# bistromath/gr-ais

Hardware: AMD Instinct MI355X
Metric: complex MS/s through corr_est->msk_timing chain; corr_est %HBM roofline (higher is better)
Workload: dtype f32

## Files before the change

### gr-ais_amd/ais_amd/_lib.py

```python
import ctypes as C
import os

_PKG = os.path.dirname(os.path.abspath(__file__))
LIB_VARIANT = os.environ.get("AISX_LIB_VARIANT", "")
LIB_PATH = os.path.join(os.path.dirname(_PKG), "lib", "libaisx_exp.so" if LIB_VARIANT == "exp" else "libaisx.so")

AISX_OK = 0
AISX_ERR_INVALID = -1
AISX_ERR_OUT_OF_RANGE = -2
AISX_ERR_HIP = -3
AISX_ERR_NO_DEVICE = -4
AISX_ERR_OVERFLOW = -5
AISX_ERR_RUNTIME = -6

AISX_FMT_CF32, AISX_FMT_CS16, AISX_FMT_CS8, AISX_FMT_CU8 = 0, 1, 2, 3
AISX_RX_ST_HDLC_OVERFLOW, AISX_RX_ST_NMEA_OVERFLOW, AISX_RX_ST_BAD_COUNT = 0x100, 0x200, 0x400
AISX_MSG_NA, AISX_MSG_STR = -(1 << 31), 48
AISX_HDLC_MAX_RULES = 16
AISX_HDLC_EV_SINGLE, AISX_HDLC_EV_PAIR, AISX_HDLC_EV_SKIP = 1, 2, 4
AISX_MLSE_ST_BAD_COUNT = 1
MLSE_BLOCK, MLSE_OVERLAP = 64, 16
AISX_MSG_FL_COMPLETE, AISX_MSG_FL_NO_LAYOUT, AISX_MSG_FL_BAD_RECORD = 1, 2, 4
AISX_NMEA_PARSE_REF_TAIL = 1
AISX_NMEAP_NAMES = ("FOUND", "KEPT", "BAD_INPUT", "LINES", "SENTENCES", "REJ_FORMAT", "REJ_CHECKSUM", "REJ_CHANNEL",
# ... 73 lines not shown
    sig("aisx_corr_set_lds_claim", i32, [vp, i32])
    sig("aisx_corr_get_lds_claim", i32, [vp, pi32, pi32])
    sig("aisx_corr_set_profiling", i32, [vp, i32])
    sig("aisx_corr_last_kernel_ms", i32, [vp, C.POINTER(C.c_float)])
    sig("aisx_corr_kernel_ms_history", i32, [vp, C.POINTER(C.c_float), i32, pi32])
    sig("aisx_corr_tags_device", i32, [vp, pvp, pvp, pi32])
    sig("aisx_corr_read_tags", i32, [vp, vp, i32, pi32, vp])
    sig("aisx_corr_read_tags_back", i32, [vp, i32, vp, i32, pi32, vp])
    sig("aisx_corr_work_host", i32, [vp, vp, vp, vp, i32, u64, vp, i32, pi32])
    sig("aisx_msk_create", i32, [pvp, f32, f32, f32, i32, i32, i32])
    sig("aisx_msk_destroy", i32, [vp])
    sig("aisx_msk_set_gain", i32, [vp, f32])
    sig("aisx_msk_get_gain", f32, [vp])
    sig("aisx_msk_set_limit", i32, [vp, f32])
    sig("aisx_msk_get_limit", f32, [vp])
    sig("aisx_msk_set_sps", i32, [vp, f32])
    sig("aisx_msk_get_sps", f32, [vp])
    sig("aisx_msk_forecast", i32, [vp, i32])
    sig("aisx_msk_out_capacity", i32, [vp])
    sig("aisx_msk_reset", i32, [vp])
    sig("aisx_msk_process_stream", i32, [vp, vp, lng, i32, vp, vp, i32, vp, vp, vp, vp, lng, vp, vp])
    sig("aisx_msk_process_stream_after", i32, [vp, vp, lng, i32, vp, vp, i32, vp, vp, vp, vp, lng, vp, vp, vp])
    sig("aisx_msk_last_status", i32, [vp, pi32, vp])
    sig("aisx_msk_restart_stats", i32, [vp, vp, vp])
    sig("aisx_msk_set_profiling", i32, [vp, i32])
    sig("aisx_msk_kernel_ms_history", i32, [vp, C.POINTER(C.c_float), i32, pi32])
    sig("aisx_msk_set_max_noutput_items", i32, [vp, i32])
    sig("aisx_msk_set_time_parallel", i32, [vp, i32, i32, i32])
    sig("aisx_msk_get_max_noutput_items", i32, [vp])
    sig("aisx_msk_set_tail_stream", i32, [vp, vp, i32])
    sig("aisx_msk_wait_tail", i32, [vp, vp])
    sig("aisx_msk_set_fused_tail", i32, [vp, i32])
    sig("aisx_msk_get_fused_tail", i32, [vp])
    sig("aisx_msk_last_tail_fused", i32, [vp])
    sig("aisx_msk_wait_prepass", i32, [vp, vp])
    sig("aisx_msk_set_head_start", i32, [vp, i32])
    sig("aisx_msk_geometry", i32, [vp, pi32, pi32])
    sig("aisx_msk_general_work_host", i32, [vp, i32, i32, vp, vp, vp, vp, vp, vp, i32, u64, i32, pi32, pi32])
    sig("aisx_freqsync_create", i32, [pvp, f64, f64, i32, i32, i32])
    sig("aisx_freqest_create", i32, [pvp, f32, i32, i32, i32])
    sig("aisx_freqest_create_n", i32, [pvp, f32, i32, i32, i32, i32])
    sig("aisx_freqsync_is_estimator_only", i32, [vp])
    sig("aisx_freqsync_geometry", i32, [vp, pi32, pi32, pi32])
    sig("aisx_freqsync_drop_ahead", i32, [vp, vp])
    sig("aisx_freqsync_destroy", i32, [vp])
    sig("aisx_freqsync_reset", i32, [vp])
    sig("aisx_freqsync_process", i32, [vp, vp, lng, i32, vp, lng, vp, lng, pi32, vp])
    sig("aisx_freqest_work", i32, [vp, vp, lng, vp, lng, i32, vp])
    sig("aisx_freqest_work_host", i32, [vp, i32, vp, vp])
    sig("aisx_freqsync_work_host", i32, [vp, vp, i32, vp, i32, vp, i32])
    sig("aisx_agc_work_host", i32, [vp, i32, vp, vp])
    sig("aisx_freqsync_agc_process", i32, [vp, vp, vp, lng, i32, vp, lng, vp, lng, pi32, vp])
    sig("aisx_freqsync_estimate_ahead", i32, [vp, vp, lng, i32, vp, vp])
    sig("aisx_agc_create", i32, [pvp, i32, f32, i32, i32])
    sig("aisx_agc_destroy", i32, [vp])
    sig("aisx_agc_geometry", i32, [vp, pi32, pi32, pi32, pi32])
    sig("aisx_agc_reset", i32, [vp])
    sig("aisx_agc_set_floor", i32, [vp, f32])
    sig("aisx_agc_set_streaming", i32, [vp, i32])
    sig("aisx_agc_set_lds_claim", i32, [vp, i32])
    sig("aisx_agc_get_lds_claim", i32, [vp, pi32, pi32])
    sig("aisx_freqsync_set_walk_lds_claim", i32, [vp, i32])
    sig("aisx_freqsync_get_walk_lds_claim", i32, [vp, pi32, pi32])
    sig("aisx_msk_placement", i32, [vp, pi32, pi32])
    sig("aisx_agc_process", i32, [vp, vp, lng, vp, lng, i32, vp])
    sig("aisx_chain_create", i32, [pvp, vp, vp, vp, vp, i32, i32, i32])
# ... 138 lines not shown
```

### gr-ais_amd/ais_amd/blocks.py

```python
import ctypes as C
import math

import numpy as np
import torch

from . import _lib
from ._lib import check

TAG_DTYPE = np.dtype([("offset", "<u8"), ("value", "<f8"), ("key", "<i4"), ("chan", "<i4")])


def _stream_ptr(stream=None):
    s = stream if stream is not None else torch.cuda.current_stream()
    return C.c_void_p(s.cuda_stream)


def _dev_c64(x, nchan):
    if not isinstance(x, torch.Tensor):
        x = torch.as_tensor(np.ascontiguousarray(x, dtype=np.complex64))
    if x.dtype != torch.complex64:
        raise TypeError("expected complex64 (gr_complex) items, got %s" % x.dtype)
    if not x.is_cuda:
        x = x.cuda()
    x = x.reshape(nchan, -1)
# ... 190 lines not shown
            else:
                width = min(width, t.shape[1])
        if prod.dim() != 1 or prod.shape[0] < self.nchan or prod.dtype != torch.int32 or not prod.is_cuda:
            raise ValueError("msk_timing_recovery_cc.work: outs['produced'] must be an int32 device tensor of nchan items")
        if stride is None:
            stride = width = cap
        if width < stride:
            raise ValueError("msk_timing_recovery_cc.work: output rows must be as wide as their stride")
        if tags_ptrs is not None:
            tptr, cptr, tcap = tags_ptrs
        elif tags_from is not None:
            tptr, cptr, tcap = tags_from.tags_device()
        else:
            tptr, cptr, tcap = None, None, 0
        check(_lib.lib().aisx_msk_process_stream(
            self._h, x.data_ptr(), x.stride(0), n, tptr, cptr, tcap,
            syms.data_ptr() if syms is not None else None, err.data_ptr() if err is not None else None,
            mu.data_ptr() if mu is not None else None, bits.data_ptr() if bits is not None else None, stride,
            prod.data_ptr(), _stream_ptr(stream)), "msk_timing_recovery_cc.work")
        return dict(syms=syms, err=err, mu=mu, bits=bits, produced=prod)

    def set_tail_stream(self, stream):
        check(_lib.lib().aisx_msk_set_tail_stream(self._h, _stream_ptr(stream) if stream is not None else None,
                                                  1 if stream is not None else 0), "set_tail_stream")

    def wait_tail(self, stream=None):
        check(_lib.lib().aisx_msk_wait_tail(self._h, _stream_ptr(stream)), "wait_tail")

    def set_fused_tail(self, on):
        check(_lib.lib().aisx_msk_set_fused_tail(self._h, 1 if on else 0), "set_fused_tail")

    def get_fused_tail(self):
        return bool(_lib.lib().aisx_msk_get_fused_tail(self._h))

    def last_tail_fused(self):
        return _lib.lib().aisx_msk_last_tail_fused(self._h) == 1

    def wait_prepass(self, stream=None):
        check(_lib.lib().aisx_msk_wait_prepass(self._h, _stream_ptr(stream)), "wait_prepass")

    def last_status(self, stream=None):
        st = C.c_int(0)
        check(_lib.lib().aisx_msk_last_status(self._h, C.byref(st), _stream_ptr(stream)), "last_status")
        return st.value

    def set_time_parallel(self, restart_points=64, join_kernel=-1, max_unit_items=0):
        check(_lib.lib().aisx_msk_set_time_parallel(self._h, int(restart_points), int(join_kernel), int(max_unit_items)),
              "set_time_parallel")

    def set_max_noutput_items(self, m):
        check(_lib.lib().aisx_msk_set_max_noutput_items(self._h, int(m)), "set_max_noutput_items")

    def max_noutput_items(self):
        return _lib.lib().aisx_msk_get_max_noutput_items(self._h)

    def set_profiling(self, on=True):
        check(_lib.lib().aisx_msk_set_profiling(self._h, 1 if on else 0), "set_profiling")

    def kernel_ms_history(self):
        buf = (C.c_float * 64)()
        n = C.c_int(0)
        check(_lib.lib().aisx_msk_kernel_ms_history(self._h, buf, 64, C.byref(n)), "kernel_ms_history")
        return [float(buf[i]) for i in range(n.value)]

    def restart_stats(self, stream=None):
        a = (C.c_longlong * 10)()
# ... 620 lines not shown
```

### gr-ais_amd/csrc/aisx_devctx.h

```cpp
#pragma once
#include <hip/hip_runtime.h>
#include "aisx_common.h"

namespace aisx {

struct DevCtx {
    static constexpr bool wave_lds_coherent = true;
    char* lds_;
    __device__ __forceinline__ int tid() const { return threadIdx.x; }
    __device__ __forceinline__ int nthreads() const { return blockDim.x; }
    __device__ __forceinline__ int bx() const { return blockIdx.x; }
    __device__ __forceinline__ int by() const { return blockIdx.y; }
    __device__ __forceinline__ char* lds() const { return lds_; }
    __device__ __forceinline__ void sync() const { __syncthreads(); }
    __device__ __forceinline__ void wave_sync() const { __builtin_amdgcn_wave_barrier(); }
    __device__ __forceinline__ void wave_lds_sync() const
    {
        asm volatile("" ::: "memory");
        __builtin_amdgcn_wave_barrier();
    }
    __device__ __forceinline__ void retire() const {}
    __device__ __forceinline__ unsigned long long ballot(bool p) const { return __builtin_amdgcn_ballot_w64(p); }
    __device__ __forceinline__ bool inv_ballot(unsigned long long m) const { return __builtin_amdgcn_inverse_ballot_w64(m); }
    typedef float v2f __attribute__((ext_vector_type(2)));
// ... 47 lines not shown
    __device__ __forceinline__ cf cmul(cf a, cf b) const
    {
        v2f m, r;
        const v2f av = tov(a), bv = tov(b);
        asm("v_pk_mul_f32 %0, %1, %2 op_sel:[0,0] op_sel_hi:[0,1]" : "=v"(m) : "v"(av), "v"(bv));
        asm("v_pk_fma_f32 %0, %1, %2, %3 op_sel:[1,1,0] op_sel_hi:[1,0,1] neg_lo:[1,0,0]" : "=v"(r) : "v"(av), "v"(bv), "v"(m));
        return tocf(r);
    }
    __device__ __forceinline__ cf cmul_conj(cf a, cf b) const
    {
        v2f m, r;
        const v2f av = tov(a), bv = tov(b);
        asm("v_pk_mul_f32 %0, %1, %2 op_sel:[0,0] op_sel_hi:[0,1] neg_hi:[1,0]" : "=v"(m) : "v"(av), "v"(bv));
        asm("v_pk_fma_f32 %0, %1, %2, %3 op_sel:[1,1,0] op_sel_hi:[1,0,1]" : "=v"(r) : "v"(av), "v"(bv), "v"(m));
        return tocf(r);
    }
    template <int W>
    __device__ __forceinline__ void pair_rows(cf v, cf& lo, cf& hi) const
    {
        static_assert(W == 16 || W == 32, "row width");
        const unsigned a = __float_as_uint(v.re), b = __float_as_uint(v.im);
        if (W == 16) {
            const auto ra = __builtin_amdgcn_permlane16_swap(a, a, false, false);
            const auto rb = __builtin_amdgcn_permlane16_swap(b, b, false, false);
            lo = mk(__uint_as_float(ra[0]), __uint_as_float(rb[0]));
            hi = mk(__uint_as_float(ra[1]), __uint_as_float(rb[1]));
        } else {
            const auto ra = __builtin_amdgcn_permlane32_swap(a, a, false, false);
            const auto rb = __builtin_amdgcn_permlane32_swap(b, b, false, false);
            lo = mk(__uint_as_float(ra[0]), __uint_as_float(rb[0]));
            hi = mk(__uint_as_float(ra[1]), __uint_as_float(rb[1]));
        }
    }
    __device__ __forceinline__ void xpose8_lane_hi(cf (&x)[8]) const
    {
        unsigned u[16];
#pragma unroll
        for (int k = 0; k < 8; k++) {
            u[2 * k] = __float_as_uint(x[k].re);
            u[2 * k + 1] = __float_as_uint(x[k].im);
        }
#pragma unroll
        for (int r = 0; r < 4; r++)
#pragma unroll
            for (int d = 0; d < 2; d++) {
                const auto q = __builtin_amdgcn_permlane32_swap(u[2 * r + d], u[2 * (r + 4) + d], false, false);
                u[2 * r + d] = q[0];
                u[2 * (r + 4) + d] = q[1];
            }
#pragma unroll
        for (int rr = 0; rr < 4; rr++) {
            const int r = (rr & 1) | ((rr & 2) << 1);
#pragma unroll
            for (int d = 0; d < 2; d++) {
                const auto q = __builtin_amdgcn_permlane16_swap(u[2 * r + d], u[2 * (r + 2) + d], false, false);
                u[2 * r + d] = q[0];
                u[2 * (r + 2) + d] = q[1];
            }
        }
#pragma unroll
        for (int r = 0; r < 8; r += 2)
#pragma unroll
            for (int d = 0; d < 2; d++) {
                const int a = (int)u[2 * r + d], b = (int)u[2 * (r + 1) + d];
                const int nb = __builtin_amdgcn_update_dpp(b, a, 0x128, 0xf, 0x3, false);
                const int na = __builtin_amdgcn_update_dpp(a, b, 0x128, 0xf, 0xc, false);
// ... 179 lines not shown
```

### gr-ais_amd/csrc/aisx_msk.hip

```cpp
#include <math.h>
#include <stdlib.h>

#include <algorithm>
#include <vector>

#include "aisx_devctx.h"
#include "aisx_msk_impl.h"
#include "aisx_plan.h"
#include "aisx_tables.h"

using namespace aisx;

template <bool AUX, bool OSPS2, int LPW>
__global__ __launch_bounds__(64 * msk_waves(LPW)) void k_msk(MskParams p)
{
    extern __shared__ __attribute__((aligned(16))) char smem[];
    DevCtx cx{ smem };
#ifndef MSK_PRIO
#define MSK_PRIO 3
#endif
    __builtin_amdgcn_s_setprio(MSK_PRIO);
    msk_body<DevCtx, AUX, OSPS2, LPW>(cx, p);
}

template <int LPW>
__global__ __launch_bounds__(64 * msk_waves(LPW)) void k_msk_ff(MskParams p)
{
    extern __shared__ __attribute__((aligned(16))) char smem[];
    DevCtx cx{ smem };
    __builtin_amdgcn_s_setprio(MSK_PRIO);
    msk_body<DevCtx, false, false, LPW, true>(cx, p);
}

__global__ __launch_bounds__(BT_T) void k_bittail(BitTailParams p)
{
    __shared__ __attribute__((aligned(16))) char smem[260 * 4];
    DevCtx cx{ smem };
    bittail_body(cx, p);
}

__global__ __launch_bounds__(64) void k_msk_headstart(unsigned ticks)
{
    const unsigned long long t0 = wall_clock64();
    for (int k = 0; k < 2048 && wall_clock64() - t0 < ticks; k++)
        __builtin_amdgcn_s_sleep(32);
}

__global__ __launch_bounds__(256) void k_msk_tagprep(TagPrepParams p)
{
    DevCtx cx{ nullptr };
    tagprep_body(cx, p);
}

int aisx::msk_launch(const MskParams& p, int nwg, hipStream_t st)
{
    typedef void (*kfn)(MskParams);
    static const kfn fns[20] = {
        k_msk<false, false, 16>, k_msk<false, true, 16>, k_msk<true, false, 16>, k_msk<true, true, 16>,
        k_msk<false, false, 32>, k_msk<false, true, 32>, k_msk<true, false, 32>, k_msk<true, true, 32>,
        k_msk<false, false, 64>, k_msk<false, true, 64>, k_msk<true, false, 64>, k_msk<true, true, 64>,
        k_msk<false, false, 8>,  k_msk<false, true, 8>,  k_msk<true, false, 8>,  k_msk<true, true, 8>,
        k_msk<false, false, 4>,  k_msk<false, true, 4>,  k_msk<true, false, 4>,  k_msk<true, true, 4>,
    };
    const int li = p.lpw == 16 ? 0 : (p.lpw == 32 ? 1 : (p.lpw == 64 ? 2 : (p.lpw == 8 ? 3 : 4)));
    const int v = li * 4 + (((p.err || p.mu_out) ? 2 : 0) | (p.osps == 2 ? 1 : 0));
    static const int pad = [] {
        const char* e = exp_env("AISX_MSK_LDS_PAD");
        return e ? atoi(e) * 1024 : 0;
    }();
    const int lds = std::min(msk_lds_bytes(p.lpw) + pad, 160 * 1024);
    kfn fn = fns[v];
    if (p.ff) {
        static const kfn ffs[5] = { k_msk_ff<16>, k_msk_ff<32>, k_msk_ff<64>, k_msk_ff<8>, k_msk_ff<4> };
        if (p.err || p.mu_out || p.osps == 2) {
            set_err("msk_launch: the join build has no err / mu ports and osps == 1");
            return AISX_ERR_INVALID;
        }
        fn = ffs[li];
    }
    int rc = ensure_dyn_lds((const void*)fn, lds, "msk_timing_recovery_cc");
    if (rc != AISX_OK)
        return rc;
    hipLaunchKernelGGL(fn, dim3(nwg), dim3(64 * msk_waves(p.lpw)), lds, st, p);
    AISX_HIPCHK(hipGetLastError());
    return AISX_OK;
}

static int msk_check_geometry(float d_sps, float gain, float limit)
{
    const float wmin = d_sps - fabsf(limit), wmax = d_sps + fabsf(limit);
    if (!(wmin >= 0.5f) || msk_forecast(d_sps, 1) + 1 > aisx_msk::carry_cap || !(2.f * wmax + 3.f * fabsf(gain) <= 32.f)) {
        set_err("msk_timing_recovery: sps/2 = %g with limit %g and gain %g is outside what the gfx950 kernel is sized for "
                "(sps/2 - |limit| >= 0.5, forecast(1) < %d items, 2 (sps/2 + |limit|) + 3 |gain| <= 32)",
                d_sps, limit, gain, aisx_msk::carry_cap);
        return AISX_ERR_INVALID;
    }
    return AISX_OK;
}
static int msk_out_cap(const aisx_msk* h)
{
    const double wmin = (double)h->d_sps - fabs((double)h->limit);
    const int tag_room = 2 * std::max(16, h->max_items / 64);
    return ((int)ceil((h->max_items + aisx_msk::carry_cap) / (2.0 * wmin)) + tag_room) * h->osps + 16;
}

static int msk_init_state(aisx_msk* h)
{
    const int nc = h->nchan;
    std::vector<float> mu(nc, 0.5f), om(nc, h->d_sps);
    AISX_HIPCHK(hipMemcpy(h->d_mu, mu.data(), sizeof(float) * nc, hipMemcpyHostToDevice));
    AISX_HIPCHK(hipMemcpy(h->d_omega, om.data(), sizeof(float) * nc, hipMemcpyHostToDevice));
// ... 145 lines not shown
{
    if (!h || max_noutput_items < 0)
        return AISX_ERR_INVALID;
    h->max_noutput = max_noutput_items;
    return AISX_OK;
}
extern "C" int aisx_msk_get_max_noutput_items(const aisx_msk* h) { return h ? h->max_noutput : AISX_ERR_INVALID; }
extern "C" int aisx_msk_out_capacity(const aisx_msk* h) { return h ? h->out_cap : AISX_ERR_INVALID; }
extern "C" int aisx_msk_reset(aisx_msk* h)
{
    if (!h)
        return AISX_ERR_INVALID;
    const int rc = msk_init_state(h);
    if (rc != AISX_OK)
        return rc;
    AISX_HIPCHK(hipDeviceSynchronize());
    return AISX_OK;
}

void aisx::msk_fill_common(aisx_msk* h, MskParams& p)
{
    msk_fill_state(h, p);
    p.osps = h->osps;
    p.ct = h->d_ct;
    p.ct_n = h->d_ct_n;
    p.ct_cap = h->ct_cap();
    p.lds_tab_off = msk_lds_taboff(h->lpw);
    p.lpw = h->lpw;
    p.lds_wave_stride = msk_lds_wave(h->lpw);
    p.tq_stride = h->lpw;
    p.tq_private = 0;
    p.lds_ring_off = msk_lds_ringoff(h->lpw);
    p.inline_tags = h->inline_tags;
    p.stream_mode = 1;
    p.gr_ninput = 0;
    p.gr_noutput = 0;
    p.ff = 0;
    p.nrst = nullptr;
    p.rst = nullptr;
    p.res = nullptr;
    p.pieces = nullptr;
    p.npieces = nullptr;
    p.ct_nc = nullptr;
}

static int msk_ct_reserve(aisx_msk* h, int need, hipStream_t st)
{
    if (h->d_ct && need <= h->ct_cap())
        return AISX_OK;
    AISX_HIPCHK(hipStreamSynchronize(st));
    const int rc = h->d_ct.reserve((size_t)h->nchan * (size_t)need);
    if (rc != AISX_OK)
        return rc;
    AISX_HIPCHK(hipDeviceSynchronize());
    return AISX_OK;
}

int aisx::msk_launch_tagprep(aisx_msk* h, const tag_rec* d_tags, const int* d_tag_counts, int tag_cap, hipStream_t st, int* d_ct_nc,
                             const msk_ctag* ctl_new, const int* ctl_new_n, int ctl_new_cap, int ctl_new_pre)
{
    const int need = aisx_msk::ctag_cap + (ctl_new ? ctl_new_cap - ctl_new_pre : (d_tags ? tag_cap : 0));
    const int rc = msk_ct_reserve(h, need, st);
    if (rc != AISX_OK)
        return rc;
    TagPrepParams t;
    t.nchan = h->nchan;
// ... 190 lines not shown
        (rc = h->ev_tail[1].ensure(hipEventDisableTiming)) != AISX_OK)
        return rc;
    h->tail_stream = (hipStream_t)tail_stream;
    h->tail_on = true;
    return AISX_OK;
}

extern "C" int aisx_msk_wait_tail(aisx_msk* h, void* stream)
{
    if (!h)
        return AISX_ERR_INVALID;
    if (h->tail_on) {
        for (int k = 0; k < 2; k++)
            if (h->ev_tail_set[k])
                AISX_HIPCHK(hipStreamWaitEvent((hipStream_t)stream, h->ev_tail[k], 0));
        if (h->last_fused && h->last_st != (hipStream_t)stream) {
            AISX_HIPCHK(hipEventRecord(h->ev_msk, h->last_st));
            AISX_HIPCHK(hipStreamWaitEvent((hipStream_t)stream, h->ev_msk, 0));
        }
    }
    return AISX_OK;
}

extern "C" int aisx_msk_set_fused_tail(aisx_msk* h, int on)
{
    if (!h)
        return AISX_ERR_INVALID;
    h->fused_tail = on != 0;
    return AISX_OK;
}
extern "C" int aisx_msk_get_fused_tail(const aisx_msk* h) { return h ? (h->fused_tail ? 1 : 0) : AISX_ERR_INVALID; }
extern "C" int aisx_msk_last_tail_fused(const aisx_msk* h) { return h ? (h->last_fused ? 1 : 0) : AISX_ERR_INVALID; }

extern "C" int aisx_msk_wait_prepass(aisx_msk* h, void* stream)
{
    if (!h)
        return AISX_ERR_INVALID;
    if (!h->ev_prep)
        return h->ev_prep.ensure(hipEventDisableTiming);
    if (h->ev_prep_set) {
        AISX_HIPCHK(hipStreamWaitEvent((hipStream_t)stream, h->ev_prep, 0));
        if (h->head_start_ticks > 0) {
            hipLaunchKernelGGL(k_msk_headstart, dim3(1), dim3(64), 0, (hipStream_t)stream, h->head_start_ticks);
            AISX_HIPCHK(hipGetLastError());
        }
    }
    return AISX_OK;
}

extern "C" int aisx_msk_set_head_start(aisx_msk* h, int microseconds)
{
    if (!h || microseconds < 0 || microseconds > 1000) {
        set_err("aisx_msk_set_head_start: 0..1000 microseconds");
        return AISX_ERR_INVALID;
    }
    int dev = 0, khz = 0;
    AISX_HIPCHK(hipGetDevice(&dev));
    if (hipDeviceGetAttribute(&khz, hipDeviceAttributeWallClockRate, dev) != hipSuccess || khz <= 0)
        khz = 100000;
    h->head_start_ticks = (unsigned)((long long)microseconds * khz / 1000);
    return AISX_OK;
}

extern "C" int aisx_msk_geometry(const aisx_msk* h, int* nchan, int* max_items)
{
    if (!h)
// ... 146 lines not shown
```

### gr-ais_amd/csrc/aisx_msk_impl.h

```cpp
#pragma once
#include <memory>
#include <vector>

#include "aisx_host.h"
#include "k_msk.h"

#pragma GCC visibility push(hidden)
namespace aisx {
struct MskTp;
struct MskTpDelete {
    void operator()(MskTp* t) const;
};
}

struct aisx_msk {
    int nchan = 0, max_items = 0, out_cap = 0, osps = 1;
    aisx::EventRing prof;
    int lpw = 64;
    int inline_tags = 1;
    float d_sps = 0, gain = 0, gain_omega = 0, limit = 0;
    static constexpr int carry_cap = aisx::MSK_CARRY_MAX, ctag_cap = 64;
    aisx::DevBuf<float> d_mu, d_omega;
    aisx::DevBuf<int> d_div;
    aisx::DevBuf<aisx::cf> d_dly1, d_dly2, d_diff1;
    aisx::DevBuf<aisx::cf> d_tprev[2];
    aisx::DevBuf<unsigned char> d_tbit[2];
    int tcur = 0;
    aisx::DevBuf<aisx::cf> d_symscratch[2];
    int callpar = 0;
    bool tail_on = false;
    hipStream_t tail_stream = nullptr;
    aisx::Event ev_msk, ev_tail[2];
    unsigned head_start_ticks = 0;
    aisx::Event ev_prep;
    bool ev_prep_set = false;
    bool ev_tail_set[2] = { false, false };
    bool fused_tail = true, last_fused = false;
    hipStream_t last_st = nullptr;
    bool tail_pend[2] = { false, false };
    aisx::DevBuf<int> d_produced2;
    aisx::DevBuf<unsigned long long> d_nread;
    aisx::DevBuf<aisx::cf> d_carry[2];
    aisx::DevBuf<int> d_carry_len[2];
    aisx::DevBuf<aisx::tag_rec> d_ctag[2];
    aisx::DevBuf<int> d_ctag_n[2];
    aisx::DevBuf<aisx::msk_ctag> d_ct;
    aisx::DevBuf<int> d_ct_n;
    int ct_cap() const { return (int)(d_ct.cap() / (size_t)nchan); }
    int cur = 0;
    aisx::DevBuf<int> d_produced, d_consumed, d_status;
    aisx::DevBuf<float> d_mmse, d_atan;
    int max_noutput = 0;
    unsigned long long total_in = 0;
    aisx::DevBuf<aisx::cf> d_st_in, d_st_blk;
    aisx::cf* d_st_sym = nullptr;
    std::vector<aisx::cf> st_host;
    aisx::DevBuf<float> d_st_err, d_st_mu;
    aisx::DevBuf<unsigned char> d_st_bits;
    aisx::DevBuf<aisx::tag_rec> d_st_tags;
    aisx::DevBuf<int> d_st_tagn;
    std::unique_ptr<aisx::MskTp, aisx::MskTpDelete> tp;
};

namespace aisx {

struct MskCall {
    const cf* in; long in_stride; int n;
    const tag_rec* tags; const int* tag_counts; int tag_cap;
    cf* syms; int* produced; long out_stride; int out_cap;
    int par; hipStream_t st;
// ... 59 lines not shown
```

### gr-ais_amd/csrc/k_msk.h

```cpp
#pragma once
#include "aisx_common.h"

namespace aisx {

enum {
    MSK_ST_INTERP_RANGE = 1,
    MSK_ST_CARRY_OVERFLOW = 2,
    MSK_ST_TAGCARRY_OVERFLOW = 4,
    MSK_ST_OUT_FULL = 8,
    MSK_ST_TAGS_TRUNCATED = 16
};
constexpr int MSK_CTN_TRUNC = 0x40000000;
constexpr int MSK_CTN_WILD = 0x20000000;
constexpr int MSK_TAG_TRIPS = 6;

constexpr int MSK_T = 64;
constexpr int MSK_RING = 256;
constexpr int MSK_SLOTS = MSK_RING + 8;
constexpr int MSK_CHUNK = 64;
constexpr int MSK_OFF = 192;
constexpr int MSK_CARRY_MAX = 128;
constexpr int MSK_PAIRS_MAX = 16;
constexpr int MSK_TAPS_PITCH = 12;
constexpr int msk_lds_ring(int lpw) { return MSK_SLOTS * lpw * 8; }
// ... 52 lines not shown
    __builtin_memcpy(&ai, &a.im, 4);
    __builtin_memcpy(&br, &b.re, 4);
    __builtin_memcpy(&bi, &b.im, 4);
    return ar == br && ai == bi;
}

struct msk_ctag { int rel; float val; };

struct __attribute__((packed, aligned(8))) cf_pair { cf a, b; };

struct MskParams {
    int nchan;
    float d_sps, gain, gain_omega, limit;
    int osps;
    float* mu; float* omega; int* div;
    cf* dly1; cf* dly2; cf* diff1;
    unsigned long long* nread;
    const cf* in; long in_stride; int n;
    const cf* carry_in; cf* carry_out; const int* carry_len_in; int* carry_len_out; int carry_cap;
    int stream_mode; int gr_ninput; int gr_noutput;
    const msk_ctag* ct; const int* ct_n; int ct_cap;
    tag_rec* ctag_out; int* ctag_n_out; int ctag_cap;
    cf* syms; float* err; float* mu_out; long out_stride; int out_cap;
    int* produced; int* consumed; int* status;
    const float* mmse;
    int lds_tab_off;
    int lds_wave_stride, tq_stride, tq_private;
    int lds_ring_off;
    int sym_al16;
    int lpw;
    int inline_tags;
    int max_noutput;
    int ff;
    const int* nrst; const mskp_rst* rst; const mskp_res* res;
    mskp_piece* pieces; int* npieces;
    const int* ct_nc;
    unsigned char* bits = nullptr; long bit_stride = 0;
    int bit_al2 = 0;
    const cf* prev_sym_in = nullptr; const unsigned char* prev_bit_in = nullptr;
    cf* prev_sym_out = nullptr; unsigned char* prev_bit_out = nullptr;
    const float* atan_tab = nullptr;
};

struct BitTailParams {
    int nchan;
    const cf* syms; long sym_stride;
    const int* produced;
    unsigned char* bits; long bit_stride;
    const cf* prev_sym_in; const unsigned char* prev_bit_in;
    cf* prev_sym_out; unsigned char* prev_bit_out;
    const float* atan_tab;
};

AISX_HD int msk_forecast(float d_sps, int noutput_items)
{
    return (int)ceil((noutput_items * d_sps * 2) + 3.0 * d_sps + 8u);
}

#ifdef MSK_EMU_STATS
extern long msk_stats[8];
#endif
template <class Ctx, bool AUX, bool OSPS2, int LPW, bool FFT = false>
AISX_DI void msk_body(Ctx& cx, const MskParams& p)
{
    static_assert(!FFT || (!AUX && !OSPS2), "the join build has no err / mu ports and osps == 1");
    constexpr int SLOT_B = LPW * 8;
    constexpr int SLOT_SH = LPW == 64 ? 9 : (LPW == 32 ? 8 : (LPW == 16 ? 7 : (LPW == 8 ? 6 : 5)));
    static_assert(LPW == 4 || LPW == 8 || LPW == 16 || LPW == 32 || LPW == 64, "channels per wave");
    typedef unsigned long long u64;
    static_assert(64 % LPW == 0, "whole waves");
    constexpr int NQ = 64 / LPW;
    constexpr int QS = MSK_CHUNK / NQ;
    const int wv = cx.tid() >> 6;
    const int l = cx.tid() & (LPW - 1);
    const int q = (cx.tid() & 63) / LPW;
    const bool owner = q == 0;
    const int cbase = cx.bx() * msk_wg_channels(LPW) + wv * LPW;
    const int c = cbase + l;
    const bool live = c < p.nchan;
    const int cc = live ? c : (p.nchan - 1);

    char* const lds0 = cx.lds();
    char* const lds = lds0 + p.lds_ring_off + wv * p.lds_wave_stride;
    cf* ring = (cf*)lds;
    float* mm = (float*)(lds0 + p.lds_tab_off);
    cf* myring = ring + l;

    for (int i = cx.tid(); i < 129 * 8; i += cx.nthreads())
        mm[(i >> 3) * MSK_TAPS_PITCH + (i & 7)] = p.mmse[i];
    if (cx.tid() < MSK_TAPS_PITCH)
        mm[MSK_ZERO_ROW * MSK_TAPS_PITCH + cx.tid()] = 0.f;
    if (cbase >= p.nchan) {
        cx.sync();
        return;
    }

    const float d_sps = p.d_sps;
    float d_mu = p.mu[cc], d_omega = p.omega[cc];
// ... 78 lines not shown
    int fin_div = 0, fin_status = 0;
    cf fin_interp = mk(0.f, 0.f), fin_diff = mk(0.f, 0.f);
    unsigned fin_worst = 0;
    int ffK = 0, ffnck = 0, cand = 0, candj = 0x7fffffff, ffnp = 0;
    int voff = 0;
    const mskp_rst* const ffrs = FF ? p.rst + (long)cc * MSKP_SMAX : nullptr;
    const mskp_res* const ffrr = FF ? p.res + (long)cc * MSKP_SMAX : nullptr;
    if (FF) {
        ffnck = p.ct_nc[cc];
        ffK = ffnck >= 0 ? p.nrst[cc] : 0;
        candj = ffK > 0 ? ffrs[0].jA + 1 + ffnck : 0x7fffffff;
    }

    char* const osym0 = p.syms ? (char*)(p.syms + (long)cbase * p.out_stride) : nullptr;
    char* const oerr0 = AUX && p.err ? (char*)(p.err + (long)cbase * p.out_stride) : nullptr;
    char* const omu0 = AUX && p.mu_out ? (char*)(p.mu_out + (long)cbase * p.out_stride) : nullptr;
    unsigned ob = (unsigned)((long)(cc - cbase) * p.out_stride) * 8u;
    constexpr bool STG = !AUX && !OSPS2 && msk_staged(LPW);
    constexpr unsigned FLQ = NQ < 8 ? NQ : 8;
    constexpr unsigned FL = 2 * FLQ;
    constexpr unsigned STG_MASK = (unsigned)((MSK_STAGE - 1) * SLOT_B);
    const unsigned obrow = ob;
    const unsigned stg_real = (unsigned)(wv * msk_lds_stage(LPW) + l * 8);
    const unsigned stg_spare = (unsigned)(p.lds_ring_off + wv * p.lds_wave_stride + p.lds_wave_stride - SLOT_B + l * 8);
    unsigned so = 0;
    unsigned nf = 0;
    struct alignas(8) cf8s { float re, im; };
    auto stage_put = [&](unsigned mask, unsigned base, cf v) {
        cf8s t;
        t.re = v.re;
        t.im = v.im;
        *(cf8s*)(lds0 + ((so & mask) | base)) = t;
        so += (unsigned)SLOT_B;
    };
    auto stage_get = [&](unsigned k) -> cf {
        const cf8s t = *(const cf8s*)(lds0 + ((((k & (unsigned)(MSK_STAGE - 1)) << SLOT_SH)) | stg_real));
        return mk(t.re, t.im);
    };
    constexpr bool FUSE = STG && !FFT;
    const bool fuse = FUSE && p.bits != nullptr;
    unsigned char* const obit0 = fuse ? p.bits + (long)cbase * p.bit_stride : nullptr;
    const unsigned bbrow = (unsigned)((long)(cc - cbase) * p.bit_stride);
    cf t_sym = mk(0.f, 0.f);
    unsigned t_bit = 0;
    if (fuse) {
        t_sym = p.prev_sym_in[cc];
        t_bit = p.prev_bit_in[cc];
    }
    struct slice_in { float y, x; bool tab; };
    auto slice_pre = [&](const cf& cur, const cf& prev, bool valid) -> slice_in {
        const cf prod = cmul_exact(cur, cconj(prev));
        const float y = prod.im, x = prod.re;
        const float ya = fabsf(y), xa = fabsf(x);
        const bool plain = (ya < 1.0e30f) && (xa < 1.0e18f) && (y >= 0.0f || ya > 1.0e-18f);
        slice_in r;
        r.y = y;
        r.x = x;
        r.tab = valid && !plain;
        return r;
    };
    auto slice_tab = [&](const slice_in& s) -> unsigned {
        const float fm = 1.57079632679489661923f * fast_atan2f_tab(s.y, s.x, p.atan_tab);
        return fm >= 0 ? 1u : 0u;
    };
    struct tail_full { enum { value = 1 }; };
    struct tail_part { enum { value = 0 }; };
// ... 652 lines not shown
                        sqE = nE;
                        sqO = nO;
                        nl_prev = skipO ? nlE : nlO;
                        last_skip = skipO;
                    }
                    cf accE, accO;
                    cx.template pair_rows<ROW>(acc, accE, accO);
                    oidx += ntrips;
                    prev_sq = sqO;
                    last_interp = last_skip ? accE : accO;
                    d_dly_diff_1 = mk(nl_prev, sqO.im * sqE.re - sqO.re * sqE.im);
                    if (!(d_mu >= 0.f && d_mu <= 1.f))
                        status |= MSK_ST_INTERP_RANGE;
                    E = cx.ballot((d_div & 1) == 0);
                    bounds(sb >> SLOT_SH);
#ifdef MSK_PROF
                    pf_n[0] += ntrips; pf_n[1]++;
#endif
                }
              }
            }
#ifdef MSK_PROF
            if (npairs == 0) { pf_fail += __builtin_readcyclecounter() - pf_a; pf_nfail++; }
#endif
            if (npairs > 0) {
              if constexpr (NQ >= 2) {
                constexpr int ROW = LPW <= 16 ? 16 : 32;
                const bool roleO = (cx.tid() & ROW) != 0;
                const unsigned rstep = (unsigned)(cx.tid() & ROW) * (unsigned)(SLOT_B / ROW);
                const unsigned pmask = roleO ? 0u : STG_MASK, pbase = roleO ? stg_spare : stg_real;
                cf sqO = prev_sq, sqE = mk(0.f, 0.f), acc = last_interp;
                float nl_prev = d_dly_diff_1.re;
                const int sb_entry = sb;
                for (int k = 0; k < npairs; k++) {
#ifdef MSK_EMU_STATS
                    if (l == 0 && q == 0) msk_stats[0]++;
#endif
                    const float m1 = d_mu + d_omega;
                    const float muO = cx.fract(m1);
                    const int adv1 = (int)m1;
                    const int sb1 = sb + adv1 * SLOT_B;
                    cf sv[8];
                    float tv[8];
                    fir_load_pair(roleO ? muO : d_mu, ring_read_off(sb, adv1, rstep, RING_M), sv, tv);
                    acc = fir_sum(sv, tv);
                    const cf sq = cmul_exact(acc, acc);
                    cf sE, s1;
                    cx.template pair_rows<ROW>(sq, sE, s1);
                    const float nlE = sE.re * sqO.re + sE.im * sqO.im;
                    const float nlO = s1.re * sE.re + s1.im * sE.im;
                    const float err = branchless_clip(nlO - nlE, 3.0f);
                    d_omega += p.gain_omega * err;
                    d_omega = d_sps + branchless_clip(d_omega - d_sps, p.limit);
                    const float mu2 = muO + p.gain * err;
                    if (OSPS2) {
                        const unsigned o = ob + (roleO ? 8u : 0u);
                        *(cf*)(osym0 + o) = acc;
                        if (AUX) {
                            if (oerr0)
                                *(float*)(oerr0 + (o >> 1)) = roleO ? err : nlE - nl_prev;
                            if (omu0)
                                *(float*)(omu0 + (o >> 1)) = roleO ? mu2 : d_mu;
                        }
                        ob += 16u;
                    } else if constexpr (STG) {
                        stage_put(pmask, pbase, acc);
                    } else {
                        if (!roleO) {
                            *(cf*)(osym0 + ob) = acc;
                            if (AUX) {
                                if (oerr0)
                                    *(float*)(oerr0 + (ob >> 1)) = nlE - nl_prev;
                                if (omu0)
                                    *(float*)(omu0 + (ob >> 1)) = d_mu;
                            }
                        }
                        ob += 8u;
                    }
                    const float m2 = mu2 + d_omega;
                    d_mu = cx.fract(m2);
                    sb = sb1 + (int)m2 * SLOT_B;
                    sqE = sE;
                    sqO = s1;
                    nl_prev = nlO;
                }
                cf accE, accO;
                cx.template pair_rows<ROW>(acc, accE, accO);
                d_div += 2 * npairs;
                oidx += OSPS2 ? 2 * npairs : npairs;
                iidx += (sb - sb_entry) >> SLOT_SH;
                prev_sq = sqO;
                last_interp = accO;
                d_dly_diff_1 = mk(nl_prev, sqO.im * sqE.re - sqO.re * sqE.im);
                if (!(d_mu >= 0.f && d_mu <= 1.f))
                    status |= MSK_ST_INTERP_RANGE;
              } else {
                const int sb_entry = sb;
                cf sqO = prev_sq, sqE = mk(0.f, 0.f), accO = last_interp;
                float nl_prev = d_dly_diff_1.re;
                for (int k = 0; k < npairs; k++) {
#ifdef MSK_EMU_STATS
                    if (l == 0) msk_stats[0]++;
#endif
                    cf svE[8], svO[8];
                    float tvE[8], tvO[8];
                    fir_load_pair(d_mu, (unsigned)sb & RING_M, svE, tvE);
                    const float m1 = d_mu + d_omega;
                    const float muO = cx.fract(m1);
                    const int sb1 = sb + (int)m1 * SLOT_B;
                    fir_load_pair(muO, (unsigned)sb1 & RING_M, svO, tvO);
                    const cf accE = fir_sum(svE, tvE);
                    const cf sE = cmul_exact(accE, accE);
                    const float nlE = sE.re * sqO.re + sE.im * sqO.im;
                    if constexpr (STG)
                        stage_put(STG_MASK, stg_real, accE);
                    else
                        *(cf*)(osym0 + ob) = accE;
                    if (AUX) {
// ... 359 lines not shown
```

### include/aisx.h

```cpp
#ifndef AISX_H
#define AISX_H

#include <stddef.h>
#include <stdint.h>

#ifdef __cplusplus
extern "C" {
#endif

#define AISX_VERSION 300

typedef struct aisx_cf32 { float re, im; } aisx_cf32;

enum {
    AISX_KEY_CORR_START = 0,
    AISX_KEY_PHASE_EST = 1,
    AISX_KEY_TIME_EST = 2,
    AISX_KEY_CORR_EST = 3,
    AISX_KEY_PORT1 = 0x100
};
typedef struct aisx_tag {
    uint64_t offset;
    double value;
    int32_t key;
// ... 57 lines not shown
float aisx_msk_get_limit(const aisx_msk* h);
int aisx_msk_set_sps(aisx_msk* h, float sps);
float aisx_msk_get_sps(const aisx_msk* h);
int aisx_msk_forecast(const aisx_msk* h, int noutput_items);
int aisx_msk_out_capacity(const aisx_msk* h);
int aisx_msk_reset(aisx_msk* h);

int aisx_msk_process_stream(aisx_msk* h, const aisx_cf32* d_in, long in_stride, int n, const aisx_tag* d_tags,
                            const int* d_tag_counts, int tag_cap, aisx_cf32* d_syms, float* d_err, float* d_mu,
                            uint8_t* d_bits, long out_stride, int* d_produced, void* stream);
int aisx_msk_process_stream_after(aisx_msk* h, const aisx_cf32* d_in, long in_stride, int n, const aisx_tag* d_tags,
                                  const int* d_tag_counts, int tag_cap, aisx_cf32* d_syms, float* d_err, float* d_mu,
                                  uint8_t* d_bits, long out_stride, int* d_produced, void* stream, void* ready_event);
enum {
    AISX_MSK_ST_INTERP_RANGE = 1,
    AISX_MSK_ST_CARRY_OVERFLOW = 2,
    AISX_MSK_ST_TAGCARRY_OVERFLOW = 4,
    AISX_MSK_ST_OUT_FULL = 8,
    AISX_MSK_ST_TAGS_TRUNCATED = 16
};
int aisx_msk_set_max_noutput_items(aisx_msk* h, int max_noutput_items);
int aisx_msk_set_time_parallel(aisx_msk* h, int restart_points_per_channel, int join_kernel, int max_unit_items);
int aisx_msk_get_max_noutput_items(const aisx_msk* h);
int aisx_msk_last_status(aisx_msk* h, int* status, void* stream);
int aisx_msk_status_device(const aisx_msk* h, const int** d_status);
int aisx_msk_restart_stats(aisx_msk* h, long long* out10, void* stream);
int aisx_msk_set_profiling(aisx_msk* h, int on);
int aisx_msk_kernel_ms_history(aisx_msk* h, float* ms, int cap, int* n);
int aisx_msk_set_tail_stream(aisx_msk* h, void* tail_stream, int enable);
int aisx_msk_wait_tail(aisx_msk* h, void* stream);
int aisx_msk_set_fused_tail(aisx_msk* h, int on);
int aisx_msk_get_fused_tail(const aisx_msk* h);
int aisx_msk_last_tail_fused(const aisx_msk* h);
int aisx_msk_wait_prepass(aisx_msk* h, void* stream);
int aisx_msk_set_head_start(aisx_msk* h, int microseconds);
int aisx_msk_general_work_host(aisx_msk* h, int noutput_items, int ninput_items, const aisx_cf32* in, aisx_cf32* out,
                               float* out_err, float* out_mu, uint8_t* out_bits, const aisx_tag* tags, int ntags,
                               uint64_t nitems_read, int in_has_lookahead, int* consumed, int* produced);

typedef struct aisx_freqsync aisx_freqsync;
int aisx_freqsync_create(aisx_freqsync** h, double samplerate, double bits_per_sec, int fftlen, int nchan,
                         int max_items);
int aisx_freqsync_destroy(aisx_freqsync* h);
int aisx_freqsync_geometry(const aisx_freqsync* h, int* nchan, int* max_items, int* fftlen);
int aisx_freqsync_drop_ahead(aisx_freqsync* h, void* stream);
int aisx_freqsync_set_walk_lds_claim(aisx_freqsync* h, int bytes);
int aisx_freqsync_get_walk_lds_claim(const aisx_freqsync* h, int* bytes, int* used_bytes);
int aisx_freqest_create(aisx_freqsync** h, float sample_rate, int data_rate, int fftlen, int max_vectors);
int aisx_freqest_create_n(aisx_freqsync** h, float sample_rate, int data_rate, int fftlen, int nchan, int max_vectors);
int aisx_freqsync_is_estimator_only(const aisx_freqsync* h);
int aisx_freqsync_reset(aisx_freqsync* h);
int aisx_freqsync_process(aisx_freqsync* h, const aisx_cf32* d_in, long in_stride, int n, aisx_cf32* d_out,
                          long out_stride, float* d_fhat, long fhat_stride, int* n_out, void* stream);
int aisx_freqsync_work_host(aisx_freqsync* h, const aisx_cf32* in, int n, aisx_cf32* out, int out_cap, float* fhat,
                            int fhat_cap);
int aisx_freqest_work(aisx_freqsync* h, const aisx_cf32* d_vecs, long vec_stride, float* d_out, long out_stride,
                      int nvec, void* stream);
int aisx_freqest_work_host(aisx_freqsync* h, int noutput_items, const aisx_cf32* in, float* out);

typedef struct aisx_agc aisx_agc;
int aisx_agc_create(aisx_agc** h, int nsamples, float reference, int nchan, int max_items);
int aisx_agc_destroy(aisx_agc* h);
int aisx_agc_geometry(const aisx_agc* h, int* nchan, int* max_items, int* nsamples, int* fused_ok);
int aisx_agc_reset(aisx_agc* h);
int aisx_agc_set_floor(aisx_agc* h, float floor_env);
int aisx_agc_set_streaming(aisx_agc* h, int on);
// ... 294 lines not shown
```

Before: 52110.

## Add hand-scheduled inline-asm pair loop for MSK timing recovery core

Adds a hand-written GCN/CDNA inline-assembly routine for the per-symbol-pair FIR interpolation, squaring and timing-error update loop. It issues its LDS reads early, overlaps them with the previous symbol's staging write, and uses packed FP32 math plus a permlane swap. A dedicated kernel instantiation with 8 lanes per wave is selected by default when the pair_core flag is set and the dispatch variant matches. The staging write is also rotated to lag one iteration so it overlaps the next loads. This aims to cut instruction count and LDS latency stalls in the serial timing loop, at the cost of fragile hand-allocated registers and hard-coded LDS offsets.

```diff
diff --git a/gr-ais_amd/ais_amd/_lib.py b/gr-ais_amd/ais_amd/_lib.py
--- a/gr-ais_amd/ais_amd/_lib.py
+++ b/gr-ais_amd/ais_amd/_lib.py
@@ -129,6 +129,8 @@
     sig("aisx_msk_wait_tail", i32, [vp, vp])
     sig("aisx_msk_set_fused_tail", i32, [vp, i32])
     sig("aisx_msk_get_fused_tail", i32, [vp])
+    sig("aisx_msk_set_pair_core", i32, [vp, i32])
+    sig("aisx_msk_get_pair_core", i32, [vp])
     sig("aisx_msk_last_tail_fused", i32, [vp])
     sig("aisx_msk_wait_prepass", i32, [vp, vp])
     sig("aisx_msk_set_head_start", i32, [vp, i32])
diff --git a/gr-ais_amd/ais_amd/blocks.py b/gr-ais_amd/ais_amd/blocks.py
--- a/gr-ais_amd/ais_amd/blocks.py
+++ b/gr-ais_amd/ais_amd/blocks.py
@@ -246,6 +246,12 @@
 
     def get_fused_tail(self):
         return bool(_lib.lib().aisx_msk_get_fused_tail(self._h))
+
+    def set_pair_core(self, mode):
+        check(_lib.lib().aisx_msk_set_pair_core(self._h, int(mode)), "set_pair_core")
+
+    def get_pair_core(self):
+        return int(_lib.lib().aisx_msk_get_pair_core(self._h))
 
     def last_tail_fused(self):
         return _lib.lib().aisx_msk_last_tail_fused(self._h) == 1
diff --git a/gr-ais_amd/csrc/aisx_devctx.h b/gr-ais_amd/csrc/aisx_devctx.h
--- a/gr-ais_amd/csrc/aisx_devctx.h
+++ b/gr-ais_amd/csrc/aisx_devctx.h
@@ -103,6 +103,99 @@
             hi = mk(__uint_as_float(ra[1]), __uint_as_float(rb[1]));
         }
     }
+    static constexpr bool has_pair_core = true;
+    struct PairK {
+        unsigned long long roleM;
+        unsigned rbase;
+        float gain_omega, d_sps, limit, gain;
+        unsigned rstep;
+        unsigned ring;
+        unsigned pmask, pbase;
+        float rnd;
+    };
+    __device__ __forceinline__ void pair_core(const PairK& k, float& mu, float& omega, int& sb, unsigned& so, unsigned& waddr, v2f& acc,
+                                              v2f& sE, v2f& s1, float& nlO) const
+    {
+        float t1, t3, t4;
+        int t2;
+        asm volatile(
+            "v_add_f32 %[t3], %[mu], %[om]\n\t"
+            "v_cvt_i32_f32 %[t2], %[t3]\n\t"
+            "v_fract_f32 %[t1], %[t3]\n\t"
+            "v_mad_u32_u24 %[t4], %[t2], %[rstep], %[sb]\n\t"
+            "v_cndmask_b32_e64 %[t3], %[mu], %[t1], %[roleM]\n\t"
+            "v_and_b32 %[t4], 0x3fc0, %[t4]\n\t"
+            "v_fmamk_f32 %[t3], %[t3], 0x43000000, %[rnd]\n\t"
+            "v_add_u32 %[t4], %[ring], %[t4]\n\t"
+            "v_mad_u32_u24 %[t3], %[t3], 48, %[rbase]\n\t"
+            "ds_read_b128 v[4:7], %[t3] offset:16\n\t"
+            "ds_read2_b64 v[8:11], %[t4] offset1:8\n\t"
+            "ds_read_b128 v[0:3], %[t3]\n\t"
+            "ds_read2_b64 v[12:15], %[t4] offset0:16 offset1:24\n\t"
+            "ds_read2_b64 v[16:19], %[t4] offset0:32 offset1:40\n\t"
+            "ds_read2_b64 v[20:23], %[t4] offset0:48 offset1:56\n\t"
+            "ds_write_b64 %[waddr], %[acc]\n\t"
+            "v_lshl_add_u32 %[sb], %[t2], 6, %[sb]\n\t"
+            "v_and_b32 %[waddr], %[so], %[pmask]\n\t"
+            "s_waitcnt lgkmcnt(5)\n\t"
+            "v_pk_mul_f32 %[acc], v[8:9], v[6:7] op_sel:[0,1] op_sel_hi:[1,1]\n\t"
+            "v_pk_mul_f32 v[8:9], v[10:11], v[6:7] op_sel_hi:[1,0]\n\t"
+            "v_pk_add_f32 %[acc], %[acc], 0 op_sel_hi:[1,0]\n\t"
+            "s_waitcnt lgkmcnt(3)\n\t"
+            "v_pk_mul_f32 v[10:11], v[12:13], v[4:5] op_sel:[0,1] op_sel_hi:[1,1]\n\t"
+            "v_pk_add_f32 %[acc], %[acc], v[8:9]\n\t"
+            "v_pk_mul_f32 v[8:9], v[14:15], v[4:5] op_sel_hi:[1,0]\n\t"
+            "v_pk_add_f32 %[acc], %[acc], v[10:11]\n\t"
+            "s_waitcnt lgkmcnt(1)\n\t"
+            "v_pk_mul_f32 v[10:11], v[16:17], v[2:3] op_sel:[0,1] op_sel_hi:[1,1]\n\t"
+            "v_pk_add_f32 %[acc], %[acc], v[8:9]\n\t"
+            "v_pk_mul_f32 v[8:9], v[18:19], v[2:3] op_sel_hi:[1,0]\n\t"
+            "v_pk_add_f32 %[acc], %[acc], v[10:11]\n\t"
+            "v_pk_mul_f32 v[10:11], v[20:21], v[0:1] op_sel:[0,1] op_sel_hi:[1,1]\n\t"
+            "v_pk_add_f32 %[acc], %[acc], v[8:9]\n\t"
+            "v_pk_mul_f32 v[8:9], v[22:23], v[0:1] op_sel_hi:[1,0]\n\t"
+            "v_pk_add_f32 %[acc], %[acc], v[10:11]\n\t"
+            "v_add_u32 %[waddr], %[pbase], %[waddr]\n\t"
+            "v_pk_add_f32 %[acc], %[acc], v[8:9]\n\t"
+            "v_add_u32 %[so], 64, %[so]\n\t"
+            "v_pk_mul_f32 v[18:19], %[acc], %[acc] op_sel:[0,0] op_sel_hi:[0,1]\n\t"
+            "v_pk_mul_f32 v[20:21], %[acc], %[acc] op_sel:[1,1] op_sel_hi:[1,0]\n\t"
+            "v_mov_b64 v[14:15], v[24:25]\n\t"
+            "v_pk_add_f32 v[16:17], v[18:19], v[20:21] neg_lo:[0,1]\n\t"
+            "v_pk_add_f32 v[24:25], v[18:19], v[20:21] neg_lo:[0,1]\n\t"
+            "s_nop 1\n\t"
+            "v_permlane16_swap_b32 v16, v24\n\t"
+            "v_permlane16_swap_b32 v17, v25\n\t"
+            "v_pk_mul_f32 v[8:9], v[16:17], v[14:15]\n\t"
+            "v_pk_mul_f32 v[10:11], v[24:25], v[16:17]\n\t"
+            "v_add_f32 v0, v8, v9\n\t"
+            "v_add_f32 %[nlO], v10, v11\n\t"
+            "v_sub_f32 v0, %[nlO], v0\n\t"
+            "v_add_f32 v1, 0x40400000, v0\n\t"
+            "v_add_f32 v2, 0xc0400000, v0\n\t"
+            "v_sub_f32_e64 v0, |v1|, |v2|\n\t"
+            "v_mul_f32 v0, 0.5, v0\n\t"
+            "v_mul_f32 v1, %[go], v0\n\t"
+            "v_mul_f32 v2, %[gain], v0\n\t"
+            "v_add_f32 v1, %[om], v1\n\t"
+            "v_add_f32 v2, %[t1], v2\n\t"
+            "v_subrev_f32 v1, %[dsps], v1\n\t"
+            "v_add_f32 v0, %[lim], v1\n\t"
+            "v_subrev_f32 v1, %[lim], v1\n\t"
+            "v_sub_f32_e64 v0, |v0|, |v1|\n\t"
+            "v_mul_f32 v0, 0.5, v0\n\t"
+            "v_add_f32 %[om], %[dsps], v0\n\t"
+            "v_add_f32 v2, v2, %[om]\n\t"
+            "v_cvt_i32_f32 v3, v2\n\t"
+            "v_fract_f32 %[mu], v2\n\t"
+            "v_lshl_add_u32 %[sb], v3, 6, %[sb]"
+            : [mu] "+v"(mu), [om] "+v"(omega), [sb] "+v"(sb), [so] "+v"(so), [waddr] "+v"(waddr), [acc] "+v"(acc), "={v[16:17]}"(sE),
+              "+{v[24:25]}"(s1), [nlO] "=&v"(nlO), [t1] "=&v"(t1), [t2] "=&v"(t2), [t3] "=&v"(t3), [t4] "=&v"(t4)
+            : [roleM] "s"(k.roleM), [rbase] "s"(k.rbase), [go] "s"(k.gain_omega), [dsps] "s"(k.d_sps), [lim] "s"(k.limit), [gain] "s"(k.gain),
+              [rstep] "v"(k.rstep), [ring] "v"(k.ring), [pmask] "v"(k.pmask), [pbase] "v"(k.pbase), [rnd] "v"(k.rnd)
+            : "memory", "v0", "v1", "v2", "v3", "v4", "v5", "v6", "v7", "v8", "v9", "v10", "v11", "v12", "v13", "v14", "v15", "v18", "v19",
+              "v20", "v21", "v22", "v23");
+    }
     __device__ __forceinline__ void xpose8_lane_hi(cf (&x)[8]) const
     {
         unsigned u[16];
diff --git a/gr-ais_amd/csrc/aisx_msk.hip b/gr-ais_amd/csrc/aisx_msk.hip
--- a/gr-ais_amd/csrc/aisx_msk.hip
+++ b/gr-ais_amd/csrc/aisx_msk.hip
@@ -30,6 +30,14 @@
     DevCtx cx{ smem };
     __builtin_amdgcn_s_setprio(MSK_PRIO);
     msk_body<DevCtx, false, false, LPW, true>(cx, p);
+}
+
+__global__ __launch_bounds__(64 * msk_waves(8)) void k_msk_core(MskParams p)
+{
+    extern __shared__ __attribute__((aligned(16))) char smem[];
+    DevCtx cx{ smem };
+    __builtin_amdgcn_s_setprio(MSK_PRIO);
+    msk_body<DevCtx, false, false, 8, false, true>(cx, p);
 }
 
 __global__ __launch_bounds__(BT_T) void k_bittail(BitTailParams p)
@@ -77,6 +85,8 @@
             return AISX_ERR_INVALID;
         }
         fn = ffs[li];
+    } else if (p.pair_core && v == 3 * 4) {
+        fn = k_msk_core;
     }
     int rc = ensure_dyn_lds((const void*)fn, lds, "msk_timing_recovery_cc");
     if (rc != AISX_OK)
@@ -288,6 +298,7 @@
     p.tq_private = 0;
     p.lds_ring_off = msk_lds_ringoff(h->lpw);
     p.inline_tags = h->inline_tags;
+    p.pair_core = h->pair_core;
     p.stream_mode = 1;
     p.gr_ninput = 0;
     p.gr_noutput = 0;
@@ -544,6 +555,15 @@
 extern "C" int aisx_msk_get_fused_tail(const aisx_msk* h) { return h ? (h->fused_tail ? 1 : 0) : AISX_ERR_INVALID; }
 extern "C" int aisx_msk_last_tail_fused(const aisx_msk* h) { return h ? (h->last_fused ? 1 : 0) : AISX_ERR_INVALID; }
 
+extern "C" int aisx_msk_set_pair_core(aisx_msk* h, int mode)
+{
+    if (!h || (mode != 0 && mode != 1))
+        return AISX_ERR_INVALID;
+    h->pair_core = mode;
+    return AISX_OK;
+}
+extern "C" int aisx_msk_get_pair_core(const aisx_msk* h) { return h ? h->pair_core : AISX_ERR_INVALID; }
+
 extern "C" int aisx_msk_wait_prepass(aisx_msk* h, void* stream)
 {
     if (!h)
diff --git a/gr-ais_amd/csrc/aisx_msk_impl.h b/gr-ais_amd/csrc/aisx_msk_impl.h
--- a/gr-ais_amd/csrc/aisx_msk_impl.h
+++ b/gr-ais_amd/csrc/aisx_msk_impl.h
@@ -36,6 +36,7 @@
     bool ev_prep_set = false;
     bool ev_tail_set[2] = { false, false };
     bool fused_tail = true, last_fused = false;
+    int pair_core = 1;
     hipStream_t last_st = nullptr;
     bool tail_pend[2] = { false, false };
     aisx::DevBuf<int> d_produced2;
diff --git a/gr-ais_amd/csrc/k_msk.h b/gr-ais_amd/csrc/k_msk.h
--- a/gr-ais_amd/csrc/k_msk.h
+++ b/gr-ais_amd/csrc/k_msk.h
@@ -108,6 +108,7 @@
     int inline_tags;
     int max_noutput;
     int ff;
+    int pair_core = 0;
     const int* nrst; const mskp_rst* rst; const mskp_res* res;
     mskp_piece* pieces; int* npieces;
     const int* ct_nc;
@@ -136,10 +137,15 @@
 #ifdef MSK_EMU_STATS
 extern long msk_stats[8];
 #endif
-template <class Ctx, bool AUX, bool OSPS2, int LPW, bool FFT = false>
+template <class Ctx, class = void>
+struct msk_has_pair_core { static constexpr bool value = false; };
+template <class Ctx>
+struct msk_has_pair_core<Ctx, decltype((void)Ctx::has_pair_core)> { static constexpr bool value = Ctx::has_pair_core; };
+template <class Ctx, bool AUX, bool OSPS2, int LPW, bool FFT = false, bool CORE = false>
 AISX_DI void msk_body(Ctx& cx, const MskParams& p)
 {
     static_assert(!FFT || (!AUX && !OSPS2), "the join build has no err / mu ports and osps == 1");
+    static_assert(!CORE || (msk_has_pair_core<Ctx>::value && !AUX && !OSPS2 && !FFT && LPW == 8), "the scheduled pair is written for this build");
     constexpr int SLOT_B = LPW * 8;
     constexpr int SLOT_SH = LPW == 64 ? 9 : (LPW == 32 ? 8 : (LPW == 16 ? 7 : (LPW == 8 ? 6 : 5)));
     static_assert(LPW == 4 || LPW == 8 || LPW == 16 || LPW == 32 || LPW == 64, "channels per wave");
@@ -284,6 +290,12 @@
         t.im = v.im;
         *(cf8s*)(lds0 + ((so & mask) | base)) = t;
         so += (unsigned)SLOT_B;
+    };
+    auto stage_at = [&](unsigned at, cf v) {
+        cf8s t;
+        t.re = v.re;
+        t.im = v.im;
+        *(cf8s*)(lds0 + at) = t;
     };
     auto stage_get = [&](unsigned k) -> cf {
         const cf8s t = *(const cf8s*)(lds0 + ((((k & (unsigned)(MSK_STAGE - 1)) << SLOT_SH)) | stg_real));
@@ -1002,6 +1014,30 @@
                 cf sqO = prev_sq, sqE = mk(0.f, 0.f), acc = last_interp;
                 float nl_prev = d_dly_diff_1.re;
                 const int sb_entry = sb;
+                constexpr bool ROT = STG && (CORE || !Ctx::wave_lds_coherent);
+                unsigned wat = stg_spare;
+              if constexpr (CORE) {
+                typename Ctx::PairK kk;
+                kk.roleM = cx.ballot(roleO);
+                kk.rbase = mm_rbase + cx.lds_addr(lds0);
+                kk.gain_omega = p.gain_omega;
+                kk.d_sps = d_sps;
+                kk.limit = p.limit;
+                kk.gain = p.gain;
+                kk.rstep = rstep;
+                kk.ring = cx.lds_addr(lds_l);
+                kk.pmask = pmask;
+                kk.pbase = pbase + cx.lds_addr(lds0);
+                kk.rnd = 12582912.0f;
+                typename Ctx::v2f a2 = Ctx::tov(acc), e2 = Ctx::tov(sqE), o2 = Ctx::tov(sqO);
+                wat += cx.lds_addr(lds0);
+                for (int k = 0; k < npairs; k++)
+                    cx.pair_core(kk, d_mu, d_omega, sb, so, wat, a2, e2, o2, nl_prev);
+                wat -= cx.lds_addr(lds0);
+                acc = Ctx::tocf(a2);
+                sqE = Ctx::tocf(e2);
+                sqO = Ctx::tocf(o2);
+              } else {
                 for (int k = 0; k < npairs; k++) {
 #ifdef MSK_EMU_STATS
                     if (l == 0 && q == 0) msk_stats[0]++;
@@ -1013,6 +1049,11 @@
                     cf sv[8];
                     float tv[8];
                     fir_load_pair(roleO ? muO : d_mu, ring_read_off(sb, adv1, rstep, RING_M), sv, tv);
+                    if constexpr (ROT) {
+                        stage_at(wat, acc);
+                        wat = (so & pmask) | pbase;
+                        so += (unsigned)SLOT_B;
+                    }
                     acc = fir_sum(sv, tv);
                     const cf sq = cmul_exact(acc, acc);
                     cf sE, s1;
@@ -1034,7 +1075,8 @@
                         }
                         ob += 16u;
                     } else if constexpr (STG) {
-                        stage_put(pmask, pbase, acc);
+                        if constexpr (!ROT)
+                            stage_put(pmask, pbase, acc);
                     } else {
                         if (!roleO) {
                             *(cf*)(osym0 + ob) = acc;
@@ -1054,6 +1096,9 @@
                     sqO = s1;
                     nl_prev = nlO;
                 }
+              }
+                if constexpr (ROT)
+                    stage_at(wat, acc);
                 cf accE, accO;
                 cx.template pair_rows<ROW>(acc, accE, accO);
                 d_div += 2 * npairs;
diff --git a/include/aisx.h b/include/aisx.h
--- a/include/aisx.h
+++ b/include/aisx.h
@@ -113,6 +113,8 @@
 int aisx_msk_set_fused_tail(aisx_msk* h, int on);
 int aisx_msk_get_fused_tail(const aisx_msk* h);
 int aisx_msk_last_tail_fused(const aisx_msk* h);
+int aisx_msk_set_pair_core(aisx_msk* h, int mode);
+int aisx_msk_get_pair_core(const aisx_msk* h);
 int aisx_msk_wait_prepass(aisx_msk* h, void* stream);
 int aisx_msk_set_head_start(aisx_msk* h, int microseconds);
 int aisx_msk_general_work_host(aisx_msk* h, int noutput_items, int ninput_items, const aisx_cf32* in, aisx_cf32* out,
```

New measurement: 53350, median of 6. 2.4% higher.
